# Keshav-Madhav/3d-spatial-sim-for-boid-and-nbody

Hardware: AMD Instinct MI355X
Metric: body-steps/sec (N-body Barnes-Hut, theta=0.5) (higher is better)
Workload: dtype f64 pair forces for the waves of 64 bodies whose densest quarter has G*rho*dt^2 > tau - and for every wave while most of the system qualifies (entered above a third of the waves, left below a quarter; library default 'auto') -, f32 pair forces with f64 sums for the others; f64 opening-test ties, f64; 1 GPU; galaxy_1m_bh; distribution=galaxy, bodies_per_gpu=1000000, bodies_total=1000000, method=barnes_hut, force_precision=auto, parallelism=single GPU

## Files before the change

### 3d-spatial-sim-for-boid-and-nbody_amd/csrc/nbmi.hip

```cpp
#include <math.h>
#include <stdarg.h>
#include <stddef.h>
#include <stdlib.h>
#include <string.h>

#include <algorithm>
#include <type_traits>
#include <utility>
#include <vector>

#include "../../include/nbmi.h"
#include "common.h"
#include "radix_hist.h"
#include "hilbert.h"
#include "visible.h"

namespace nbmi {
static thread_local char g_err[512] = "";
void set_error(const char *fmt, ...) {
    va_list ap;
    va_start(ap, fmt);
    vsnprintf(g_err, sizeof(g_err), fmt, ap);
    va_end(ap);
}
// ... 125 lines not shown

template <bool kHilbert, typename TD, typename TN>
__device__ __forceinline__ uint64_t key_word(double px, double py, double pz, double &cx, double &cy, double &cz, double &hs,
                                             unsigned &st, const TD *hd, const TN *hn) {
    uint64_t kk = 0;
    for (int l = 0; l < 21; l++) {
        const double q = hs * 0.5;
        const bool bx = px >= cx, by = py >= cy, bz = pz >= cz;
        cx = bx ? cx + q : cx - q;
        cy = by ? cy + q : cy - q;
        cz = bz ? cz + q : cz - q;
        hs = q;
        const unsigned oct = (bx ? 1u : 0u) | (by ? 2u : 0u) | (bz ? 4u : 0u);
        if (kHilbert) {
            kk = (kk << 3) | (uint64_t)((hd[st] >> (3u * oct)) & 7u);
            st = (unsigned)(hn[st] >> (5u * oct)) & 31u;
        } else {
            kk = (kk << 3) | (uint64_t)oct;
        }
    }
    return kk;
}

__device__ __noinline__ uint64_t key_low_word(bool hilbert, double px, double py, double pz, double bounds) {
    double cx = 0.0, cy = 0.0, cz = 0.0, hs = bounds;
    unsigned st = 0u;
    if (hilbert) {
        (void)key_word<true>(px, py, pz, cx, cy, cz, hs, st, nbmi::kHilDigit, nbmi::kHilNext);
        return key_word<true>(px, py, pz, cx, cy, cz, hs, st, nbmi::kHilDigit, nbmi::kHilNext);
    }
    (void)key_word<false>(px, py, pz, cx, cy, cz, hs, st, nbmi::kHilDigit, nbmi::kHilNext);
    return key_word<false>(px, py, pz, cx, cy, cz, hs, st, nbmi::kHilDigit, nbmi::kHilNext);
}
__device__ __forceinline__ uint64_t low_word_of(const uint64_t *__restrict__ key_lo, const Bodies &cur, uint32_t b, int hilbert,
                                                const TreeInfo *info) {
    return key_lo ? key_lo[b] : key_low_word(hilbert != 0, cur.x[b], cur.y[b], cur.z[b], info->bounds);
}

constexpr int kKeysHistBlock = 1024, kKeysHistMaxGrid = 512;
constexpr int kKeysHistCounters = 4096;
static inline bool fused_hist_pays(int64_t n) { return n <= 2097152; }
static inline int keys_hist_grid(int64_t n) {
    const int64_t g = (n + 2 * kKeysHistBlock - 1) / (2 * kKeysHistBlock);
    return (int)(g < 1 ? 1 : (g > kKeysHistMaxGrid ? kKeysHistMaxGrid : g));
}
template <bool kHilbert, bool kLean>
__device__ __forceinline__ uint64_t keys_of_body(int64_t i, const double *__restrict__ x, const double *__restrict__ y,
                                                 const double *__restrict__ z, double bounds, uint64_t *__restrict__ key_hi,
                                                 uint64_t *__restrict__ key_lo, uint32_t *__restrict__ idx,
                                                 uint64_t *__restrict__ packed, int shift, const uint32_t *hd, const uint64_t *hn) {
    const double px = x[i], py = y[i], pz = z[i];
    double cx = 0.0, cy = 0.0, cz = 0.0, hs = bounds;
    uint64_t k[2];
    unsigned st = 0u;
    k[0] = key_word<kHilbert>(px, py, pz, cx, cy, cz, hs, st, hd, hn);
// ... 122 lines not shown
    }
    const int64_t s = lo_ok, e = hi_bad;
    if (r == s && e - s > 64 && !(!kPacked && dead_rank && srt[e - 1] == ~0ull)) atomicMax(&info->max_run, (int)(e - s < 0x7fffffff ? e - s : 0x7fffffff));
    uint64_t la = key_lo ? key_lo[p] : 0ull;
    bool have_la = key_lo != nullptr;
    int64_t before = 0;
    for (int64_t j = s; j < e; j++) {
        const uint32_t pj = body(j);
        const uint64_t hj = upper(j, pj);
        if (hj != h) {
            before += hj < h ? 1 : 0;
        } else {
            if (pj == p) continue;
            if (!have_la) { la = low_word_of(key_lo, cur, p, hilbert, info); have_la = true; }
            const uint64_t lj = low_word_of(key_lo, cur, pj, hilbert, info);
            before += (lj < la || (lj == la && pj < p)) ? 1 : 0;
        }
    }
    perm_out[s + before] = p;
    hi_out[s + before] = h;
}

constexpr int kScanItems = 8;
constexpr int kScanTile = kBlock * kScanItems;
constexpr int kSubShift = 11;
static_assert(kScanTile == (1 << kSubShift), "a sub-tile is one workgroup's tile");

struct dd {
    double h, l;
};
__device__ __forceinline__ dd dd_add(const dd &a, const dd &b) {
    const double s = a.h + b.h;
    const double bb = s - a.h;
    double e = (a.h - (s - bb)) + (b.h - bb);
    e += a.l + b.l;
    const double h = s + e;
    return dd{h, e - (h - s)};
}
__device__ __forceinline__ double dd_diff(const dd &a, const dd &b) {
    const dd d = dd_add(a, dd{-b.h, -b.l});
    return d.h + d.l;
}

__device__ __forceinline__ int64_t pex_at(const int32_t *__restrict__ PexL, const int32_t *__restrict__ subPex, int64_t r) {
    return (int64_t)subPex[r >> kSubShift] + PexL[r];
}

struct Mom4 {
    double m, x, y, z;
    int c;
};
__device__ __forceinline__ Mom4 operator+(const Mom4 &a, const Mom4 &b) { return Mom4{a.m + b.m, a.x + b.x, a.y + b.y, a.z + b.z, a.c + b.c}; }
__device__ __forceinline__ Mom4 lane_up(const Mom4 &v, int d) {
    return Mom4{__shfl_up(v.m, d), __shfl_up(v.x, d), __shfl_up(v.y, d), __shfl_up(v.z, d), __shfl_up(v.c, d)};
}

template <int CTRL>
__device__ __forceinline__ float dpp_f(float v) {
    return __int_as_float(__builtin_amdgcn_update_dpp(0, __float_as_int(v), CTRL, 0xF, 0xF, false));
}
__device__ __forceinline__ float add_f(float a, float b) { return a + b; }

template <bool kLean>
__global__ __launch_bounds__(kBlock) void k_gather_scan(Bodies cur, const uint32_t *__restrict__ perm,
                                                        const uint64_t *__restrict__ hi_s, const uint64_t *__restrict__ key_lo,
                                                        int64_t n, double G, float4 *__restrict__ posm_s,
                                                        double4 *__restrict__ p64_s , uint64_t *__restrict__ lo_s,
                                                        int32_t *__restrict__ delta, double4 *__restrict__ S,
                                                        int32_t *__restrict__ PexL, double4 *__restrict__ sub_tot,
                                                        int32_t *__restrict__ sub_cnt, unsigned char *__restrict__ wave_flag,
                                                        int32_t *__restrict__ sub_flag, float dens_thr, float edge_floor,
                                                        const TreeInfo *__restrict__ info, int hilbert) {
    __shared__ int wflag[kBlock / 64];
    int nflag = 0;
    __shared__ int dl[kBlock + 1];
    const int t = threadIdx.x, lane = t & 63, w = t >> 6;
    Mom4 carry{0.0, 0.0, 0.0, 0.0, 0};
#pragma unroll 1
    for (int k = 0; k < kScanItems; k++) {
        const int64_t r0 = (int64_t)blockIdx.x * kScanTile + (int64_t)k * kBlock;
        if (r0 > n) break;
        const int64_t r = r0 + t;
        Mom4 v{0.0, 0.0, 0.0, 0.0, 0};
        int d = -1;
        uint64_t h = 0, l = 0;
        float fx = 0.f, fy = 0.f, fz = 0.f;
        if (r < n) {
            const uint32_t j = perm[r];
            const double x = cur.x[j], y = cur.y[j], z = cur.z[j], gm = G * cur.m[j];
            fx = (float)x; fy = (float)y; fz = (float)z;
            posm_s[r] = make_float4((float)x, (float)y, (float)z, (float)gm);
            if (p64_s) p64_s[r] = make_double4(x, y, z, gm);
            h = hi_s[r];
            if (!kLean) {
                l = key_lo[j];
                lo_s[r] = l;
            }
            if (r + 1 < n) {
                const uint64_t hn = hi_s[r + 1];
                uint64_t ln = 0ull;
                uint64_t lr = l;
                if (hn == h) {
                    if (kLean) lr = low_word_of(nullptr, cur, j, hilbert, info);
                    ln = kLean ? low_word_of(nullptr, cur, perm[r + 1], hilbert, info) : key_lo[perm[r + 1]];
                }
                d = cpl_digits(h, lr, hn, ln);
            }
            delta[r] = d;
            v = Mom4{gm, gm * x, gm * y, gm * z, 0};
        }
        if (wave_flag) {
            const bool have = r < n;
            const float big = 3.0e38f;
            float lox = have ? fx : big, hix = have ? fx : -big, loy = have ? fy : big, hiy = have ? fy : -big;
            float loz = have ? fz : big, hiz = have ? fz : -big, gsum = have ? (float)v.m : 0.f;
#define NBMI_ROW16(V, OP)                      \
    V = OP(V, dpp_f<0xB1>(V));                 \
    V = OP(V, dpp_f<0x4E>(V));                 \
    V = OP(V, dpp_f<0x141>(V));                \
    V = OP(V, dpp_f<0x140>(V));
            NBMI_ROW16(lox, fminf) NBMI_ROW16(hix, fmaxf) NBMI_ROW16(loy, fminf) NBMI_ROW16(hiy, fmaxf)
            NBMI_ROW16(loz, fminf) NBMI_ROW16(hiz, fmaxf) NBMI_ROW16(gsum, add_f)
#undef NBMI_ROW16
            const float vol = fmaxf(hix - lox, edge_floor) * fmaxf(hiy - loy, edge_floor) * fmaxf(hiz - loz, edge_floor);
            float dens = gsum > 0.f ? gsum / vol : 0.f;
            dens = fmaxf(dens, __shfl_xor(dens, 16));
            dens = fmaxf(dens, __shfl_xor(dens, 32));
            const int flag = dens > dens_thr ? 1 : 0;
            if (lane == 0) {
                if (r0 + 64 * w < n) wave_flag[(r0 >> 6) + w] = (unsigned char)flag;
                nflag += (r0 + 64 * w < n) ? flag : 0;
            }
        }
        dl[t + 1] = d;
        if (t == 0) {
            int dp = -1;
            if (r > 0 && r < n) {
                const uint64_t hp = hi_s[r - 1];
                uint64_t lp = 0ull, lr = l;
                if (hp == h) {
                    if (kLean) lr = low_word_of(nullptr, cur, perm[r], hilbert, info);
                    lp = kLean ? low_word_of(nullptr, cur, perm[r - 1], hilbert, info) : key_lo[perm[r - 1]];
                }
                dp = cpl_digits(hp, lp, h, lr);
            }
            dl[0] = dp;
        }
        __syncthreads();
        if (r < n) {
            const int dp = dl[t];
            v.c = d > dp ? d - dp : 0;
        }
        const scan::Scanned<Mom4> sc = scan::block_scan<kBlock>(v, carry, scan::Sum());
        carry = carry + sc.total;
        if (r <= n) {
            S[r] = make_double4(sc.excl.m, sc.excl.x, sc.excl.y, sc.excl.z);
            PexL[r] = sc.excl.c;
        }
    }
    if (wave_flag) {
        if (lane == 0) wflag[w] = nflag;
        __syncthreads();
    }
    if (t == 0) {
        sub_tot[blockIdx.x] = make_double4(carry.m, carry.x, carry.y, carry.z);
        sub_cnt[blockIdx.x] = carry.c;
        if (wave_flag) sub_flag[blockIdx.x] = wflag[0] + wflag[1] + wflag[2] + wflag[3];
    }
}

constexpr int kSubScanThreads = 1024;
struct SubVal {
    dd m, x, y, z;
    long long c;
};
__device__ __forceinline__ SubVal operator+(const SubVal &a, const SubVal &b) {
    return SubVal{dd_add(a.m, b.m), dd_add(a.x, b.x), dd_add(a.y, b.y), dd_add(a.z, b.z), a.c + b.c};
}
__device__ __forceinline__ SubVal sub_zero() { return SubVal{{0.0, 0.0}, {0.0, 0.0}, {0.0, 0.0}, {0.0, 0.0}, 0}; }
__device__ __forceinline__ dd dd_shfl_up(const dd &v, int d) { return dd{__shfl_up(v.h, d), __shfl_up(v.l, d)}; }
__device__ __forceinline__ SubVal lane_up(const SubVal &v, int d) {
    return SubVal{dd_shfl_up(v.m, d), dd_shfl_up(v.x, d), dd_shfl_up(v.y, d), dd_shfl_up(v.z, d), __shfl_up(v.c, d)};
}
constexpr int kAll64Enter = 333, kAll64Leave = 250;
__host__ __device__ inline int all64_rule(int prev, long long ask, long long waves, int enter_pm, int leave_pm) {
    return prev ? (1000 * ask >= (long long)leave_pm * waves ? 1 : 0) : (1000 * ask > (long long)enter_pm * waves ? 1 : 0);
}
__global__ void k_set_all64(TreeInfo *info, int v) { info->force_all64 = v; }

__global__ __launch_bounds__(kSubScanThreads) void k_scan_subtiles(const double4 *__restrict__ sub_tot,
// ... 46 lines not shown
                                              double &M, double &mx, double &my, double &mz) {
    const double4 s0 = S[r], s1 = S[e];
    M = s1.x - s0.x; mx = s1.y - s0.y; my = s1.z - s0.z; mz = s1.w - s0.w;
    const int64_t ur = r >> kSubShift, ue = e >> kSubShift;
    if (ue != ur) {
        const Moment a = T[ur], b = T[ue];
        M += dd_diff(dd{b.m, b.ml}, dd{a.m, a.ml});
        mx += dd_diff(dd{b.x, b.xl}, dd{a.x, a.xl});
        my += dd_diff(dd{b.y, b.yl}, dd{a.y, a.yl});
        mz += dd_diff(dd{b.z, b.zl}, dd{a.z, a.zl});
    }
}

__device__ __forceinline__ void write_sentinel(Node *__restrict__ nodes, int32_t *__restrict__ node_ref, int64_t total,
                                               int64_t link_base = 0) {
    Node sn;
    sn.cx = sn.cy = sn.cz = 1.0e30f;
    sn.gm = 0.f; sn.s2t = 0.f;
    sn.next_off = (unsigned)(total + link_base) * kNodeBytes;
    nodes[total] = sn;
    if (node_ref) node_ref[total] = -1;
}

template <int TILE>
__global__ __launch_bounds__(kBlock) void k_emit_tile(const int32_t *__restrict__ delta, const int32_t *__restrict__ PexL,
                                                      const int32_t *__restrict__ subPex, const double4 *__restrict__ S,
                                                      const Moment *__restrict__ T, const float4 *__restrict__ posm_s,
                                                      const uint64_t *__restrict__ hi_s,
                                                      const uint64_t *__restrict__ lo_s, int64_t n, int64_t capacity,
                                                      double eps, double inv_theta2, Node *__restrict__ nodes,
                                                      Node64 *__restrict__ nodes64, uint8_t *__restrict__ node_level,
                                                      int32_t *__restrict__ node_ref, double4 *__restrict__ diag64,
                                                      NodeD *__restrict__ nodesd , Bodies cur,
                                                      const uint32_t *__restrict__ perm, double G, TreeInfo *info, int hilbert,
                                                      int64_t link_base ) {
    __shared__ uint8_t tree[2 * TILE];
    __shared__ uint8_t dprev;
    __shared__ uint32_t cells[(2 * TILE)];
    const int t = threadIdx.x;
    const int64_t base = (int64_t)blockIdx.x * TILE;
    const int64_t total = n + pex_at(PexL, subPex, n);
    if (blockIdx.x == 0 && t == 0) {
        info->num_nodes = total;
        info->walk_nodes = total;
        info->band2 = 2u * band_half_ulps(__longlong_as_double((long long)info->maxabs_bits), eps);
        if (total + 1 > capacity) {
            info->error = 1;
            if (info->sticky_error == 0) {
                info->sticky_error = 1;
                info->sticky_nodes = total;
            }
        } else {
            write_sentinel(nodes, node_ref, total, link_base);
            if (nodesd) nodesd[total] = NodeD{1.0e30, 1.0e30, 1.0e30, 0.0, 0.0f, (unsigned)(total + link_base) * kNodeDBytes};
        }
    }
    if (total + 1 > capacity) return;
    for (int i = t; i < TILE; i += kBlock) {
        const int64_t r = base + i;
        tree[TILE + i] = (uint8_t)((r < n ? delta[r] : -1) + 1);
    }
    if (t == 0) dprev = (uint8_t)((base > 0 ? delta[base - 1] : -1) + 1);
    __syncthreads();
    for (int width = TILE / 2; width >= 1; width >>= 1) {
        for (int i = t; i < width; i += kBlock) {
            const uint8_t a = tree[2 * (width + i)], b = tree[2 * (width + i) + 1];
            tree[width + i] = a < b ? a : b;
        }
        __syncthreads();
    }
    const int64_t q_tile = pex_at(PexL, subPex, base < n ? base : n);
    const int64_t tile_end = base + TILE < n ? base + TILE : n;
    const int64_t ncell = pex_at(PexL, subPex, tile_end) - q_tile;
    const int64_t nnode = (tile_end - base) + ncell;
    const int64_t idx0 = base + q_tile;
    const double bounds = info->bounds;
    const unsigned bandk = band_half_ulps(__longlong_as_double((long long)info->maxabs_bits), eps);
    for (int64_t c0 = 0; c0 < nnode; c0 += (2 * TILE)) {
        for (int i = t; i < TILE; i += kBlock) {
            const int64_t r = base + i;
            if (r >= n) break;
            const int d = (int)tree[TILE + i] - 1;
            const int dp = (int)(i > 0 ? tree[TILE + i - 1] : dprev) - 1;
            const int cnt = d > dp ? d - dp : 0;
            const int64_t s0 = i + (pex_at(PexL, subPex, r) - q_tile) - c0;
            for (int k = 0; k <= cnt; k++) {
                const int64_t c = s0 + k;
                if (c >= 0 && c < (2 * TILE)) cells[c] = ((uint32_t)i << 6) | (uint32_t)k;
            }
        }
        __syncthreads();
        const int64_t here = nnode - c0 < (2 * TILE) ? nnode - c0 : (2 * TILE);
        for (int64_t c = t; c < here; c += kBlock) {
            const uint32_t cl = cells[c];
            const int i = (int)(cl >> 6), k = (int)(cl & 63u);
            const int64_t r = base + i;
            const int64_t idx = idx0 + c0 + c;
            const int d = (int)tree[TILE + i] - 1;
            const int dp = (int)(i > 0 ? tree[TILE + i - 1] : dprev) - 1;
            const int cnt = d > dp ? d - dp : 0;
            if (k == cnt) {
                const float4 p = posm_s[r];
                Node lf;
                lf.cx = p.x; lf.cy = p.y; lf.cz = p.z; lf.gm = p.w;
                lf.s2t = 0.0f;
                lf.next_off = (unsigned)(idx + 1 + link_base) * kNodeBytes;
                nodes[idx] = lf;
                if (diag64) {
                    const uint32_t j = perm[r];
                    diag64[idx] = make_double4(cur.x[j], cur.y[j], cur.z[j], G * cur.m[j]);
                }
                if (nodesd) {
                    const uint32_t j = perm[r];
                    nodesd[idx] = NodeD{cur.x[j], cur.y[j], cur.z[j], G * cur.m[j], 0.0f, (unsigned)(idx + 1 + link_base) * kNodeDBytes};
                }
                if (node_ref) {
                    node_ref[idx] = (int32_t)r;
                    node_level[idx] = (uint8_t)((d > dp ? d : dp) + 1);
                }
                continue;
            }
            const int lev = dp + 1 + k;
            unsigned h = (unsigned)(TILE + i);
            bool found = false;
            for (;;) {
                if ((int)tree[h] <= lev) { found = true; break; }
                while ((h & 1u) && h > 1u) h >>= 1;
                if (h == 1u) break;
                h += 1u;
            }
            int64_t e;
            if (found) {
                while (h < (unsigned)TILE) {
                    h <<= 1;
                    if ((int)tree[h] > lev) h += 1u;
                }
                e = base + (int64_t)(h - (unsigned)TILE) + 1;
            } else {
                const uint64_t kh = hi_s[r];
                const bool deep = lev > 21;
                const uint64_t kl = lo_s ? lo_s[r] : (deep ? low_word_of(nullptr, cur, perm[r], hilbert, info) : 0ull);
                auto reaches = [&](int64_t u) {
                    const uint64_t hu = hi_s[u];
                    const uint64_t lu = lo_s ? lo_s[u] : (deep && hu == kh ? low_word_of(nullptr, cur, perm[u], hilbert, info) : 0ull);
                    return cpl_digits(kh, kl, hu, lu) >= lev;
                };
                int64_t ok = base + TILE - 1, bad, step = 1;
                for (;;) {
                    const int64_t u = ok + step;
                    if (u >= n) { bad = n; break; }
                    if (reaches(u)) { ok = u; step <<= 1; }
                    else { bad = u; break; }
                }
                while (bad - ok > 1) {
                    const int64_t mid = ok + ((bad - ok) >> 1);
                    if (reaches(mid)) ok = mid; else bad = mid;
                }
                e = bad;
            }
            double M, mx, my, mz;
            range_moments(S, T, r, e, M, mx, my, mz);
            double cx = 0.0, cy = 0.0, cz = 0.0;
            if (M > 0.0) { cx = mx / M; cy = my / M; cz = mz / M; }
            const double size = ldexp(bounds, 1 - lev);
            Node nd;
            nd.cx = (float)cx; nd.cy = (float)cy; nd.cz = (float)cz;
            nd.gm = (float)M;
            const float s2t = (float)(size * size * inv_theta2);
            nd.s2t = __int_as_float(__float_as_int(s2t) + (int)bandk);
            const int64_t nxt = e + pex_at(PexL, subPex, e) + link_base;
            nd.next_off = (unsigned)nxt * kNodeBytes;
            nodes[idx] = nd;
            if (nodesd) nodesd[idx] = NodeD{cx, cy, cz, M, __int_as_float(__float_as_int(s2t) + (int)kBand64), (unsigned)nxt * kNodeDBytes};
            nodes64[idx] = Node64{cx, cy, cz, ldexp(bounds, -lev)};
            if (diag64) diag64[idx] = make_double4(cx, cy, cz, M);
            if (node_ref) {
                node_ref[idx] = (int32_t)r;
                node_level[idx] = (uint8_t)lev;
            }
        }
        __syncthreads();
    }
}

__global__ __launch_bounds__(kBlock) void k_max_level(const int32_t *__restrict__ delta, int64_t n, TreeInfo *info) {
    __shared__ int red[kBlock / 64];
    int m = -1;
    for (int64_t i = (int64_t)blockIdx.x * kBlock + threadIdx.x; i < n; i += (int64_t)gridDim.x * kBlock) {
        const int d = delta[i];
        m = d > m ? d : m;
    }
#pragma unroll
    for (int o = 32; o > 0; o >>= 1) {
        const int other = __shfl_xor(m, o);
        m = other > m ? other : m;
    }
    if ((threadIdx.x & 63) == 0) red[threadIdx.x >> 6] = m;
    __syncthreads();
    if (threadIdx.x == 0) {
        for (int w = 1; w < kBlock / 64; w++) m = red[w] > m ? red[w] : m;
        atomicMax(&info->max_level, m + 1);
// ... 2808 lines not shown
    uint32_t *vis_slot = nullptr, *vis_tiles = nullptr;
    int xcd_chunk = 0;
    int xcd_balance = 1;
    int *xcd_bounds = nullptr;
    unsigned *wave_cycles = nullptr;
    unsigned char *wave_flag = nullptr;
    int32_t *sub_flag = nullptr;
    double step_dt = 0.0;
    double uniform_gm = -1.0;
    double max_gm = 0.0;
    int owner_all64 = -1;
    double owner_dt = 0.0;
    int balance_blocks = 0;
    hipStream_t side = nullptr;
    hipEvent_t ev_walked = nullptr, ev_cut = nullptr;
    bool cut_pending = false;
    int walk_block = kBlock;
    bool keys_lean = true;
    bool lean_build = false;
    bool sort_packed = true;
    uint64_t *packed = nullptr, *packed_s = nullptr;
    nbmi::RadixConfig sort_cfg;
    int sort_fused_hist = -1;
    int sort_bits = 0;
    bool maxabs_fused = false;
    bool fuse_maxabs = true;
    bool hilbert = true;
    double *diag_phi = nullptr;
    int32_t *diag_cnt = nullptr;
    double *diag_part = nullptr;
    long long *diag_partc = nullptr;
    double4 *diag_pot = nullptr;
    TreeInfo *side_info = nullptr;
    double *knn_r2 = nullptr, *knn_mass = nullptr;
    double4 *knn_rows = nullptr;
    unsigned long long *knn_evals = nullptr;
    int32_t *fof_parent = nullptr, *fof_root = nullptr, *fof_minid = nullptr, *fof_cnt = nullptr;
    uint32_t *fof_wleaf = nullptr;
    unsigned long long *fof_counters = nullptr;
    bool fof_ready = false, fof_cat_ready = false;
    uint32_t *fof_key_s = nullptr, *fof_rank = nullptr, *fof_rank_s = nullptr, *fof_tiles = nullptr;
    int32_t *fof_hpos = nullptr, *fof_slot = nullptr, *fof_qhead = nullptr;
    char *fof_sort_tmp = nullptr;
    size_t fof_sort_bytes = 0;
    double *fof_last = nullptr, *fof_first = nullptr;
    int64_t fof_row_cap = 0;
// ... 184 lines not shown
                k_keys_hist<decltype(h)::value, decltype(l)::value><<<grid, kKeysHistBlock, 0, st>>>(
                    cur.x, cur.y, cur.z, n, s->info, s->key_hi, s->key_lo, pk, shift, hist, rounds);
            }
            else
                k_keys<decltype(h)::value, decltype(l)::value><<<nblocks(n), kBlock, 0, st>>>(cur.x, cur.y, cur.z, n, s->info, s->key_hi,
                                                                                             s->key_lo, s->idx, dead, pk, shift);
        });
    });
    if (req.timed) NBMI_HIP_CHECK(hipEventRecord(s->ev[1], st));
    if (packed) {
        NBMI_HIP_CHECK(nbmi::radix_sort_keys_u64(s->tmp_sort, s->tmp_sort_bytes, s->packed, s->packed_s, (size_t)n, kPackIdxBits,
                                                 kPackIdxBits + s->sort_bits, st, s->sort_cfg, fused));
        k_tiefix<true><<<nblocks(n), kBlock, 0, st>>>(s->packed_s, s->key_hi, key_lo, nullptr, shift, s->perm, s->hi_s, n, s->info, cur, hil);
    } else {
        NBMI_HIP_CHECK(nbmi::radix_sort_pairs_u64(s->tmp_sort, s->tmp_sort_bytes, s->key_hi, s->hi_s, s->idx, s->perm,
                                                  (size_t)n, shift, 63, st));
        k_tiefix<false><<<nblocks(n), kBlock, 0, st>>>(s->hi_s, nullptr, key_lo, s->perm, shift, s->idx, s->key_hi, n, s->info, cur, hil,
                                                       dead ? s->let_scan : nullptr, n - n_live);
        std::swap(s->perm, s->idx);
        std::swap(s->hi_s, s->key_hi);
    }
    s->t_hi = s->hi_s;
    if (req.timed) NBMI_HIP_CHECK(hipEventRecord(s->ev[2], st));
    with_bool(lean, [&](auto l) {
        k_gather_scan<decltype(l)::value><<<(int)((n_live + 1 + kScanTile - 1) / kScanTile), kBlock, 0, st>>>(
            cur, s->perm, s->hi_s, key_lo, n_live, s->G, s->posm_s, s->p64_s, lean ? nullptr : s->lo_s, s->delta, s->S, s->Pex,
            s->sub_tot, s->sub_cnt, auto_prec(s) ? s->wave_flag : nullptr, s->sub_flag,
            auto_prec(s) ? (float)(s->prec_tau / (s->step_dt * s->step_dt)) : 0.f, (float)s->softening, s->info, hil);
    });
    return 0;
}

int enqueue_global_tree(nbmi_sim *s, bool aux = true, double4 *diag = nullptr) {
    const int64_t n = s->nt;
    hipStream_t st = s->stream;
    const int64_t nsub = (n + 1 + kScanTile - 1) / kScanTile;
    k_scan_subtiles<<<1, kSubScanThreads, 0, st>>>(s->sub_tot, s->sub_cnt, nsub, s->T, s->subPex,
                                                   auto_prec(s) ? s->sub_flag : nullptr, (n + 63) / 64, s->all64_enter_pm, s->all64_leave_pm, s->info);
    const double inv_theta2 = s->theta > 0.0 ? 1.0 / (s->theta * s->theta) : INFINITY;
    const int64_t ob = s->own_base;
    const bool quad = s->multipole == NBMI_MULTIPOLE_QUADRUPOLE;
    if (quad) {
        aux = true;
        if (!diag) diag = s->quad_pot;
    }
    with_int<kEmitTileSmall, kEmitTile>(n <= kEmitSmallBodies ? kEmitTileSmall : kEmitTile, [&](auto tile) {
        constexpr int kTile = decltype(tile)::value;
        k_emit_tile<kTile><<<(int)((n + kTile - 1) / kTile), kBlock, 0, st>>>(
            s->delta, s->Pex, s->subPex, s->S, s->T, s->t_posm, s->t_hi, s->lean_build ? nullptr : s->t_lo, n,
            s->own_node_rows, s->softening, inv_theta2, s->nodes + ob, s->nodes64 + ob, aux ? s->node_level : nullptr,
            aux ? s->node_ref : nullptr, diag, s->force_prec != 1 && s->nodesd ? s->nodesd + ob : nullptr,
            s->buf[s->curbuf], s->perm, s->G, s->info, s->hilbert ? 1 : 0, ob);
    });
    if (quad && n > 0) {
        k_max_level<<<64, kBlock, 0, st>>>(s->delta, n, s->info);
        for (int lev = kMaxLevel; lev >= 0; lev--)
            k_quad_level<<<kQuadGrid, kBlock, 0, st>>>(s->nodes, s->node_level, diag, s->info, lev, s->quad_work, s->nodesq);
    }
    NBMI_HIP_CHECK(hipGetLastError());
    return 0;
}

int enqueue_tree(nbmi_sim *s, const BuildRequest &req = {}) {
    if (s->owner) {
        nbmi::set_error("this handle is in owner mode: use the nbmi_owner_* calls");
        return NBMI_ERR_ARG;
    }
    const DtScope dt_scope(s, req.step_dt);
    const bool timed = req.timing != BuildTiming::kNone;
    if (req.timing == BuildTiming::kAll) NBMI_HIP_CHECK(hipEventRecord(s->ev[0], s->stream));
    if (int rc = enqueue_maxabs(s)) return rc;
    const bool lean = s->keys_lean && req.step_dt > 0.0 && !req.aux && s->multipole != NBMI_MULTIPOLE_QUADRUPOLE;
    if (int rc = enqueue_local_sort(s, SortRequest{timed, lean})) return rc;
    if (int rc = enqueue_global_tree(s, req.aux, req.diag_rows)) return rc;
    if (timed) NBMI_HIP_CHECK(hipEventRecord(s->ev[3], s->stream));
// ... 304 lines not shown
    if (s->h_info) (void)hipHostFree(s->h_info);
    if (s->stream) (void)hipStreamDestroy(s->stream);
    delete s;
}

static const char *multipole_refusal(const nbmi_sim *s) {
    if (s->method != NBMI_METHOD_BARNES_HUT) return "direct N^2 handles have no cells";
    if (s->owner) return "owner-mode handles are not supported (the exchanged tree rows carry no second moments)";
    if (s->shard_begin != 0 || s->shard_end != s->n) return "sharded handles are not supported (the exchange rows carry no second moments)";
    return nullptr;
}

static void read_env_knobs(nbmi_sim *s) {
    if (const char *e = getenv("NBMI_XCD_CHUNK")) s->xcd_chunk = atoi(e);
    if (const char *e = getenv("NBMI_XCD_BALANCE")) s->xcd_balance = atoi(e);
    if (const char *e = getenv("NBMI_SPLIT_WAVES")) s->split_max_waves = atoll(e);
    if (const char *e = getenv("NBMI_WALK_PAIR")) s->walk_pair = atoi(e);
    if (const char *e = getenv("NBMI_FUSE_MAXABS")) s->fuse_maxabs = atoi(e) != 0;
    if (const char *e = getenv("NBMI_HILBERT")) s->hilbert = atoi(e) != 0;
    if (const char *e = getenv("NBMI_SORT_PACKED")) s->sort_packed = atoi(e) != 0;
    if (const char *e = getenv("NBMI_SORT_DIGIT_BITS")) s->sort_cfg.digit_bits = atoi(e);
    if (const char *e = getenv("NBMI_SORT_THREADS")) s->sort_cfg.threads = atoi(e);
    if (const char *e = getenv("NBMI_SORT_FUSED_HIST")) s->sort_fused_hist = atoi(e) != 0 ? 1 : 0;
    if (const char *e = getenv("NBMI_KEYS_LEAN")) s->keys_lean = atoi(e) != 0;
    if (const char *e = getenv("NBMI_PAIRS_CELLS")) s->pair_cells = atoi(e) != 0;
    if (const char *e = getenv("NBMI_FORCE_PREC")) {
        const int v = atoi(e);
        if (v >= 0 && v <= 2) s->force_prec = v;
    }
    if (const char *e = getenv("NBMI_PREC_TAU")) s->prec_tau = atof(e);
    if (const char *e = getenv("NBMI_MULTIPOLE")) {
        if (!strcmp(e, "quadrupole") || !strcmp(e, "1")) s->multipole_env = NBMI_MULTIPOLE_QUADRUPOLE;
    }
    if (const char *e = getenv("NBMI_ALL64_ENTER")) s->all64_enter_pm = (int)(1000.0 * atof(e) + 0.5);
    if (const char *e = getenv("NBMI_ALL64_LEAVE")) s->all64_leave_pm = (int)(1000.0 * atof(e) + 0.5);
    if (const char *e = getenv("NBMI_SORT_BITS")) {
        const int b = atoi(e);
        if (b >= 8 && b <= 63) s->sort_bits = b;
    }
    if (const char *e = getenv("NBMI_WALK_BLOCK")) {
        const int b = atoi(e);
        if (b == 64 || b == 128 || b == 256) s->walk_block = b;
    }
}

static nbmi_sim *create_failed(nbmi_sim *s) {
    std::string keep = nbmi::get_error();
    nbmi_destroy(s);
    nbmi::set_error("%s", keep.c_str());
    return nullptr;
}

static int create_impl(nbmi_sim *s, const double *pos, const double *vel, const double *mass) {
    const int64_t n = s->n;
    const int64_t c = s->cap > n ? s->cap : n;
    if (!nbmi::radix_config_ok(s->sort_cfg)) {
        nbmi::set_error("NBMI_SORT_DIGIT_BITS must be 8 or 10 and NBMI_SORT_THREADS 256, 512 or 1024 (got %d, %d)", s->sort_cfg.digit_bits,
                        s->sort_cfg.threads);
        return NBMI_ERR_ARG;
    }
    NBMI_HIP_CHECK(hipSetDevice(s->device));
    NBMI_HIP_CHECK(hipStreamCreateWithFlags(&s->stream, hipStreamNonBlocking));
    for (auto &e : s->ev) NBMI_HIP_CHECK(hipEventCreate(&e));
    if (alloc_bodies(s, &s->buf[0], c) || alloc_bodies(s, &s->buf[1], c)) return -2;
    if (dev_alloc(s, &s->posm_s, c) || dev_alloc(s, &s->colors, 3 * (c ? c : 1)) || dev_alloc(s, &s->info, 1)) return -2;
    void *stage = nullptr;
    NBMI_HIP_CHECK(hipMalloc(&stage, (size_t)(c ? c : 1) * 7 * sizeof(double)));
    s->allocs.push_back(stage);
    s->stage = stage;
    NBMI_HIP_CHECK(hipMemsetAsync(s->info, 0, sizeof(TreeInfo), s->stream));
    NBMI_HIP_CHECK(hipMemsetAsync(s->colors, 0, (size_t)(c ? c : 1) * 3 * sizeof(float), s->stream));
    if (s->method == NBMI_METHOD_BARNES_HUT) {
        s->node_capacity = node_rows_for(c) + s->node_extra;
        const int64_t own_rows = node_rows_for(c);
        if (dev_alloc(s, &s->key_hi, c) || dev_alloc(s, &s->key_lo, c) || dev_alloc(s, &s->hi_s, c) ||
            dev_alloc(s, &s->lo_s, c) ||
            (s->sort_packed && !s->owner && (dev_alloc(s, &s->packed, c) || dev_alloc(s, &s->packed_s, c))) || (s->owner && dev_alloc(s, &s->p64_s, c)) || dev_alloc(s, &s->idx, c) ||
            dev_alloc(s, &s->perm, c) || dev_alloc(s, &s->delta, c) || dev_alloc(s, &s->Pex, c + 1) ||
// ... 1701 lines not shown
```

### 3d-spatial-sim-for-boid-and-nbody_amd/csrc/scan.h

```cpp
#pragma once
#include <hip/hip_runtime.h>
#include <stdint.h>

namespace scan {

struct Sum {
    template <class T>
    __device__ T operator()(const T &a, const T &b) const { return a + b; }
};
struct Min {
    template <class T>
    __device__ T operator()(const T &a, const T &b) const { return b < a ? b : a; }
};

template <class T>
__device__ __forceinline__ T lane_up(const T &v, int d) { return __shfl_up(v, d); }

template <class T>
struct Scanned {
    T excl, incl, total;
};

template <int NT, class T, class Op>
__device__ __forceinline__ Scanned<T> block_scan(const T &v, const T &seed, Op op) {
    static_assert(NT % 64 == 0 && NT <= 1024, "whole waves of one workgroup");
    __shared__ T wave_total[NT / 64];
    const int lane = threadIdx.x & 63;
    const int wave = __builtin_amdgcn_readfirstlane(threadIdx.x >> 6);
    T inc = v;
#pragma unroll
    for (int d = 1; d < 64; d <<= 1) {
        const T below = lane_up(inc, d);
        if (lane >= d) inc = op(below, inc);
    }
    if (lane == 63) wave_total[wave] = inc;
    __syncthreads();
    T front = seed, total = wave_total[0];
#pragma unroll
    for (int q = 0; q < NT / 64; q++) {
        if (q < wave) front = op(front, wave_total[q]);
        if (q > 0) total = op(total, wave_total[q]);
    }
    __syncthreads();
    inc = op(front, inc);
    T ex = lane_up(inc, 1);
    if (lane == 0) ex = front;
    return Scanned<T>{ex, inc, total};
}

constexpr int kScanThreads = 1024;
template <class TI, class TO, class Op>
static __global__ __launch_bounds__(kScanThreads) void k_scan_values(const TI *in, TO *out, int64_t m, int64_t stride,
                                                                    TO ident, Op op) {
    in += (int64_t)blockIdx.y * stride;
    out += (int64_t)blockIdx.y * stride;
    TO carry = ident;
    for (int64_t base = 0; base < m; base += kScanThreads) {
        const int64_t i = base + threadIdx.x;
        const TO v = i < m ? (TO)in[i] : ident;
        const Scanned<TO> s = block_scan<kScanThreads>(v, carry, op);
        if (i < m) out[i] = s.excl;
        carry = op(carry, s.total);
    }
    if (threadIdx.x == 0) out[m] = carry;
}

template <int NT, class TO>
__device__ __forceinline__ int64_t tile_slot(const TO *__restrict__ tile_off, unsigned c) {
    return (int64_t)tile_off[blockIdx.x] + block_scan<NT>(c, 0u, Sum()).excl;
}
// ... 47 lines not shown
```

Baseline: 516.0 million body-steps/s.

## Widen gather-scan to 1024 threads and drop shared delta exchange

The gather/scan kernel is templated on block size and defaults to 1024 threads, so one sub-tile is covered in two rounds instead of eight. It uses a new round-aware block scan that keeps wave totals in shared memory across rounds. The previous-delta exchange through shared memory and its extra barrier is replaced by a lane shuffle, with lane 0 computing its own predecessor. The low Morton/Hilbert word is recomputed by an inlined single 42-level loop, the emit kernel takes a packed argument struct with wave-uniform scalars, and occupancy hints are added. This risks higher register pressure and a different floating-point summation order in the moment scan.

```diff
diff --git a/3d-spatial-sim-for-boid-and-nbody_amd/csrc/nbmi.hip b/3d-spatial-sim-for-boid-and-nbody_amd/csrc/nbmi.hip
--- a/3d-spatial-sim-for-boid-and-nbody_amd/csrc/nbmi.hip
+++ b/3d-spatial-sim-for-boid-and-nbody_amd/csrc/nbmi.hip
@@ -171,15 +171,30 @@
     return kk;
 }
 
-__device__ __noinline__ uint64_t key_low_word(bool hilbert, double px, double py, double pz, double bounds) {
+__device__ __forceinline__ uint64_t key_low_word_inl(bool hilbert, double px, double py, double pz, double bounds) {
     double cx = 0.0, cy = 0.0, cz = 0.0, hs = bounds;
     unsigned st = 0u;
-    if (hilbert) {
-        (void)key_word<true>(px, py, pz, cx, cy, cz, hs, st, nbmi::kHilDigit, nbmi::kHilNext);
-        return key_word<true>(px, py, pz, cx, cy, cz, hs, st, nbmi::kHilDigit, nbmi::kHilNext);
-    }
-    (void)key_word<false>(px, py, pz, cx, cy, cz, hs, st, nbmi::kHilDigit, nbmi::kHilNext);
-    return key_word<false>(px, py, pz, cx, cy, cz, hs, st, nbmi::kHilDigit, nbmi::kHilNext);
+    uint64_t kk = 0;
+#pragma unroll 1
+    for (int l = 0; l < 42; l++) {
+        const double q = hs * 0.5;
+        const bool bx = px >= cx, by = py >= cy, bz = pz >= cz;
+        cx = bx ? cx + q : cx - q;
+        cy = by ? cy + q : cy - q;
+        cz = bz ? cz + q : cz - q;
+        hs = q;
+        const unsigned oct = (bx ? 1u : 0u) | (by ? 2u : 0u) | (bz ? 4u : 0u);
+        unsigned digit = oct;
+        if (hilbert) {
+            digit = (nbmi::kHilDigit[st] >> (3u * oct)) & 7u;
+            st = (unsigned)(nbmi::kHilNext[st] >> (5u * oct)) & 31u;
+        }
+        kk = (kk << 3) | (uint64_t)digit;
+    }
+    return kk & 0x7fffffffffffffffull;
+}
+__device__ __noinline__ uint64_t key_low_word(bool hilbert, double px, double py, double pz, double bounds) {
+    return key_low_word_inl(hilbert, px, py, pz, bounds);
 }
 __device__ __forceinline__ uint64_t low_word_of(const uint64_t *__restrict__ key_lo, const Bodies &cur, uint32_t b, int hilbert,
                                                 const TreeInfo *info) {
@@ -348,6 +363,7 @@
 }
 
 constexpr int kScanItems = 8;
+constexpr int kScanWide = 1024;
 constexpr int kScanTile = kBlock * kScanItems;
 constexpr int kSubShift = 11;
 static_assert(kScanTile == (1 << kSubShift), "a sub-tile is one workgroup's tile");
@@ -380,6 +396,13 @@
 __device__ __forceinline__ Mom4 lane_up(const Mom4 &v, int d) {
     return Mom4{__shfl_up(v.m, d), __shfl_up(v.x, d), __shfl_up(v.y, d), __shfl_up(v.z, d), __shfl_up(v.c, d)};
 }
+__device__ __forceinline__ double readlane_f64(double v, int src) {
+    return __hiloint2double(__builtin_amdgcn_readlane(__double2hiint(v), src), __builtin_amdgcn_readlane(__double2loint(v), src));
+}
+__device__ __forceinline__ Mom4 lane_get(const Mom4 &v, int src) {
+    return Mom4{readlane_f64(v.m, src), readlane_f64(v.x, src), readlane_f64(v.y, src), readlane_f64(v.z, src),
+                __builtin_amdgcn_readlane(v.c, src)};
+}
 
 template <int CTRL>
 __device__ __forceinline__ float dpp_f(float v) {
@@ -387,53 +410,60 @@
 }
 __device__ __forceinline__ float add_f(float a, float b) { return a + b; }
 
-template <bool kLean>
-__global__ __launch_bounds__(kBlock) void k_gather_scan(Bodies cur, const uint32_t *__restrict__ perm,
-                                                        const uint64_t *__restrict__ hi_s, const uint64_t *__restrict__ key_lo,
-                                                        int64_t n, double G, float4 *__restrict__ posm_s,
-                                                        double4 *__restrict__ p64_s , uint64_t *__restrict__ lo_s,
-                                                        int32_t *__restrict__ delta, double4 *__restrict__ S,
-                                                        int32_t *__restrict__ PexL, double4 *__restrict__ sub_tot,
-                                                        int32_t *__restrict__ sub_cnt, unsigned char *__restrict__ wave_flag,
-                                                        int32_t *__restrict__ sub_flag, float dens_thr, float edge_floor,
-                                                        const TreeInfo *__restrict__ info, int hilbert) {
-    __shared__ int wflag[kBlock / 64];
+template <bool kLean, int NT>
+__global__ __launch_bounds__(NT) __attribute__((amdgpu_waves_per_eu(kLean || NT == kScanWide ? 8 : 7, 8))) void k_gather_scan(
+    Bodies cur, const uint32_t *__restrict__ perm, const uint64_t *__restrict__ hi_s, const uint64_t *__restrict__ key_lo,
+    int64_t n, double G, float4 *__restrict__ posm_s, double4 *__restrict__ p64_s ,
+    uint64_t *__restrict__ lo_s, int32_t *__restrict__ delta, double4 *__restrict__ S, int32_t *__restrict__ PexL,
+    double4 *__restrict__ sub_tot, int32_t *__restrict__ sub_cnt, unsigned char *__restrict__ wave_flag,
+    int32_t *__restrict__ sub_flag, float dens_thr, float edge_floor, const TreeInfo *__restrict__ info, int hilbert) {
+    __shared__ int wflag[NT / 64];
     int nflag = 0;
-    __shared__ int dl[kBlock + 1];
     const int t = threadIdx.x, lane = t & 63, w = t >> 6;
     Mom4 carry{0.0, 0.0, 0.0, 0.0, 0};
 #pragma unroll 1
-    for (int k = 0; k < kScanItems; k++) {
-        const int64_t r0 = (int64_t)blockIdx.x * kScanTile + (int64_t)k * kBlock;
+    for (int k = 0; k < kScanTile / NT; k++) {
+        const int64_t r0 = (int64_t)blockIdx.x * kScanTile + (int64_t)k * NT;
         if (r0 > n) break;
         const int64_t r = r0 + t;
         Mom4 v{0.0, 0.0, 0.0, 0.0, 0};
-        int d = -1;
-        uint64_t h = 0, l = 0;
+        int d = -1, dp = -1;
         float fx = 0.f, fy = 0.f, fz = 0.f;
         if (r < n) {
+            const bool nxt = r + 1 < n, prv = lane == 0 && r > 0;
             const uint32_t j = perm[r];
+            const uint64_t h = hi_s[r], hn = nxt ? hi_s[r + 1] : 0ull, hp = prv ? hi_s[r - 1] : 0ull;
             const double x = cur.x[j], y = cur.y[j], z = cur.z[j], gm = G * cur.m[j];
-            fx = (float)x; fy = (float)y; fz = (float)z;
-            posm_s[r] = make_float4((float)x, (float)y, (float)z, (float)gm);
-            if (p64_s) p64_s[r] = make_double4(x, y, z, gm);
-            h = hi_s[r];
+            uint64_t l = 0ull;
             if (!kLean) {
                 l = key_lo[j];
                 lo_s[r] = l;
             }
-            if (r + 1 < n) {
-                const uint64_t hn = hi_s[r + 1];
-                uint64_t ln = 0ull;
-                uint64_t lr = l;
-                if (hn == h) {
-                    if (kLean) lr = low_word_of(nullptr, cur, j, hilbert, info);
-                    ln = kLean ? low_word_of(nullptr, cur, perm[r + 1], hilbert, info) : key_lo[perm[r + 1]];
+            fx = (float)x; fy = (float)y; fz = (float)z;
+            posm_s[r] = make_float4((float)x, (float)y, (float)z, (float)gm);
+            if (p64_s) p64_s[r] = make_double4(x, y, z, gm);
+            v = Mom4{gm, gm * x, gm * y, gm * z, 0};
+            const bool eq_n = nxt && hn == h, eq_p = prv && hp == h;
+            uint64_t ln = 0ull, lp = 0ull;
+            if (eq_n || eq_p) {
+                if (kLean) {
+                    const bool hil = hilbert != 0;
+                    const double bounds = info->bounds;
+#pragma unroll 1
+                    for (int side = -1; side < 2; side++) {
+                        if (!(side < 0 ? eq_p : (side > 0 ? eq_n : true))) continue;
+                        const uint32_t b = perm[r + side];
+                        const uint64_t lb = key_low_word_inl(hil, cur.x[b], cur.y[b], cur.z[b], bounds);
+                        if (side < 0) lp = lb; else if (side > 0) ln = lb; else l = lb;
+                    }
+                } else {
+                    if (eq_n) ln = key_lo[perm[r + 1]];
+                    if (eq_p) lp = key_lo[perm[r - 1]];
                 }
-                d = cpl_digits(h, lr, hn, ln);
             }
+            if (nxt) d = cpl_digits(h, l, hn, ln);
+            if (prv) dp = cpl_digits(hp, lp, h, l);
             delta[r] = d;
-            v = Mom4{gm, gm * x, gm * y, gm * z, 0};
         }
         if (wave_flag) {
             const bool have = r < n;
@@ -458,27 +488,12 @@
                 nflag += (r0 + 64 * w < n) ? flag : 0;
             }
         }
-        dl[t + 1] = d;
-        if (t == 0) {
-            int dp = -1;
-            if (r > 0 && r < n) {
-                const uint64_t hp = hi_s[r - 1];
-                uint64_t lp = 0ull, lr = l;
-                if (hp == h) {
-                    if (kLean) lr = low_word_of(nullptr, cur, perm[r], hilbert, info);
-                    lp = kLean ? low_word_of(nullptr, cur, perm[r - 1], hilbert, info) : key_lo[perm[r - 1]];
-                }
-                dp = cpl_digits(hp, lp, h, lr);
-            }
-            dl[0] = dp;
-        }
-        __syncthreads();
-        if (r < n) {
-            const int dp = dl[t];
-            v.c = d > dp ? d - dp : 0;
-        }
-        const scan::Scanned<Mom4> sc = scan::block_scan<kBlock>(v, carry, scan::Sum());
-        carry = carry + sc.total;
+        const int d_below = __shfl_up(d, 1);
+        if (lane != 0) dp = d_below;
+        if (r < n) v.c = d > dp ? d - dp : 0;
+        const scan::ScannedRounds<Mom4> sc =
+            scan::block_scan_rounds256<NT, kScanTile / NT>(v, Mom4{0.0, 0.0, 0.0, 0.0, 0}, scan::Sum(), k);
+        carry = sc.carry;
         if (r <= n) {
             S[r] = make_double4(sc.excl.m, sc.excl.x, sc.excl.y, sc.excl.z);
             PexL[r] = sc.excl.c;
@@ -491,7 +506,11 @@
     if (t == 0) {
         sub_tot[blockIdx.x] = make_double4(carry.m, carry.x, carry.y, carry.z);
         sub_cnt[blockIdx.x] = carry.c;
-        if (wave_flag) sub_flag[blockIdx.x] = wflag[0] + wflag[1] + wflag[2] + wflag[3];
+        if (wave_flag) {
+            int f = 0;
+            for (int q = 0; q < NT / 64; q++) f += wflag[q];
+            sub_flag[blockIdx.x] = f;
+        }
     }
 }
 
@@ -584,76 +603,126 @@
     if (node_ref) node_ref[total] = -1;
 }
 
+struct EmitArgs {
+    const int32_t *delta, *PexL, *subPex;
+    const double4 *S;
+    const Moment *T;
+    const float4 *posm_s;
+    const uint64_t *hi_s, *lo_s;
+    int64_t n, capacity;
+    double eps, inv_theta2;
+    Node *nodes;
+    Node64 *nodes64;
+    uint8_t *node_level;
+    int32_t *node_ref;
+    double4 *diag64;
+    NodeD *nodesd;
+    Bodies cur;
+    const uint32_t *perm;
+    double G;
+    TreeInfo *info;
+    int hilbert;
+    int64_t link_base;
+};
+
+__device__ __forceinline__ int64_t first_lane(int64_t v) {
+    const unsigned lo = __builtin_amdgcn_readfirstlane((unsigned)v), hi = __builtin_amdgcn_readfirstlane((unsigned)((uint64_t)v >> 32));
+    return (int64_t)(((uint64_t)hi << 32) | lo);
+}
+
+__device__ __forceinline__ void emit_header(const EmitArgs &a, int64_t total) {
+    TreeInfo *info = a.info;
+    info->num_nodes = total;
+    info->walk_nodes = total;
+    info->band2 = 2u * band_half_ulps(__longlong_as_double((long long)info->maxabs_bits), a.eps);
+    if (total + 1 > a.capacity) {
+        info->error = 1;
+        if (info->sticky_error == 0) {
+            info->sticky_error = 1;
+            info->sticky_nodes = total;
+        }
+    } else {
+        write_sentinel(a.nodes, a.node_ref, total, a.link_base);
+        if (a.nodesd) a.nodesd[total] = NodeD{1.0e30, 1.0e30, 1.0e30, 0.0, 0.0f, (unsigned)(total + a.link_base) * kNodeDBytes};
+    }
+}
+
+__device__ __forceinline__ int64_t cell_end_beyond(const EmitArgs &a, int64_t r, int lev, int64_t ok) {
+    const uint64_t *hi_s = a.hi_s, *lo_s = a.lo_s;
+    const int64_t n = a.n;
+    const uint64_t kh = hi_s[r];
+    const bool deep = lev > 21;
+    auto recomputed = [&](int64_t u) {
+        const uint32_t b = a.perm[u];
+        return key_low_word_inl(a.hilbert != 0, a.cur.x[b], a.cur.y[b], a.cur.z[b], a.info->bounds);
+    };
+    const uint64_t kl = lo_s ? lo_s[r] : (deep ? recomputed(r) : 0ull);
+    auto reaches = [&](int64_t u) {
+        const uint64_t hu = hi_s[u];
+        const uint64_t lu = lo_s ? lo_s[u] : (deep && hu == kh ? recomputed(u) : 0ull);
+        return cpl_digits(kh, kl, hu, lu) >= lev;
+    };
+    int64_t bad, step = 1;
+    for (;;) {
+        const int64_t u = ok + step;
+        if (u >= n) { bad = n; break; }
+        if (reaches(u)) { ok = u; step <<= 1; }
+        else { bad = u; break; }
+    }
+    while (bad - ok > 1) {
+        const int64_t mid = ok + ((bad - ok) >> 1);
+        if (reaches(mid)) ok = mid; else bad = mid;
+    }
+    return bad;
+}
+
 template <int TILE>
-__global__ __launch_bounds__(kBlock) void k_emit_tile(const int32_t *__restrict__ delta, const int32_t *__restrict__ PexL,
-                                                      const int32_t *__restrict__ subPex, const double4 *__restrict__ S,
-                                                      const Moment *__restrict__ T, const float4 *__restrict__ posm_s,
-                                                      const uint64_t *__restrict__ hi_s,
-                                                      const uint64_t *__restrict__ lo_s, int64_t n, int64_t capacity,
-                                                      double eps, double inv_theta2, Node *__restrict__ nodes,
-                                                      Node64 *__restrict__ nodes64, uint8_t *__restrict__ node_level,
-                                                      int32_t *__restrict__ node_ref, double4 *__restrict__ diag64,
-                                                      NodeD *__restrict__ nodesd , Bodies cur,
-                                                      const uint32_t *__restrict__ perm, double G, TreeInfo *info, int hilbert,
-                                                      int64_t link_base ) {
+__global__ __launch_bounds__(kBlock) __attribute__((amdgpu_waves_per_eu(5, 8))) void k_emit_tile(const EmitArgs a) {
     __shared__ uint8_t tree[2 * TILE];
     __shared__ uint8_t dprev;
     __shared__ uint32_t cells[(2 * TILE)];
     const int t = threadIdx.x;
+    const int64_t n = a.n;
     const int64_t base = (int64_t)blockIdx.x * TILE;
-    const int64_t total = n + pex_at(PexL, subPex, n);
-    if (blockIdx.x == 0 && t == 0) {
-        info->num_nodes = total;
-        info->walk_nodes = total;
-        info->band2 = 2u * band_half_ulps(__longlong_as_double((long long)info->maxabs_bits), eps);
-        if (total + 1 > capacity) {
-            info->error = 1;
-            if (info->sticky_error == 0) {
-                info->sticky_error = 1;
-                info->sticky_nodes = total;
-            }
-        } else {
-            write_sentinel(nodes, node_ref, total, link_base);
-            if (nodesd) nodesd[total] = NodeD{1.0e30, 1.0e30, 1.0e30, 0.0, 0.0f, (unsigned)(total + link_base) * kNodeDBytes};
-        }
-    }
-    if (total + 1 > capacity) return;
+    const int64_t total = first_lane(n + pex_at(a.PexL, a.subPex, n));
+    if (blockIdx.x == 0 && t == 0) emit_header(a, total);
+    if (total + 1 > a.capacity) return;
     for (int i = t; i < TILE; i += kBlock) {
         const int64_t r = base + i;
-        tree[TILE + i] = (uint8_t)((r < n ? delta[r] : -1) + 1);
-    }
-    if (t == 0) dprev = (uint8_t)((base > 0 ? delta[base - 1] : -1) + 1);
+        tree[TILE + i] = (uint8_t)((r < n ? a.delta[r] : -1) + 1);
+    }
+    if (t == 0) dprev = (uint8_t)((base > 0 ? a.delta[base - 1] : -1) + 1);
     __syncthreads();
     for (int width = TILE / 2; width >= 1; width >>= 1) {
         for (int i = t; i < width; i += kBlock) {
-            const uint8_t a = tree[2 * (width + i)], b = tree[2 * (width + i) + 1];
-            tree[width + i] = a < b ? a : b;
+            const uint8_t a0 = tree[2 * (width + i)], a1 = tree[2 * (width + i) + 1];
+            tree[width + i] = a0 < a1 ? a0 : a1;
         }
         __syncthreads();
     }
-    const int64_t q_tile = pex_at(PexL, subPex, base < n ? base : n);
+    const int64_t q_tile = first_lane(pex_at(a.PexL, a.subPex, base < n ? base : n));
     const int64_t tile_end = base + TILE < n ? base + TILE : n;
-    const int64_t ncell = pex_at(PexL, subPex, tile_end) - q_tile;
-    const int64_t nnode = (tile_end - base) + ncell;
+    const int ncell = (int)(first_lane(pex_at(a.PexL, a.subPex, tile_end)) - q_tile);
+    const int nnode = (int)(tile_end - base) + ncell;
     const int64_t idx0 = base + q_tile;
-    const double bounds = info->bounds;
-    const unsigned bandk = band_half_ulps(__longlong_as_double((long long)info->maxabs_bits), eps);
-    for (int64_t c0 = 0; c0 < nnode; c0 += (2 * TILE)) {
+    const double bounds = a.info->bounds;
+    const unsigned bandk = band_half_ulps(__longlong_as_double((long long)a.info->maxabs_bits), a.eps);
+    for (int c0 = 0; c0 < nnode; c0 += (2 * TILE)) {
         for (int i = t; i < TILE; i += kBlock) {
             const int64_t r = base + i;
             if (r >= n) break;
             const int d = (int)tree[TILE + i] - 1;
             const int dp = (int)(i > 0 ? tree[TILE + i - 1] : dprev) - 1;
             const int cnt = d > dp ? d - dp : 0;
-            const int64_t s0 = i + (pex_at(PexL, subPex, r) - q_tile) - c0;
+            const int s0 = i + (int)(pex_at(a.PexL, a.subPex, r) - q_tile) - c0;
             for (int k = 0; k <= cnt; k++) {
-                const int64_t c = s0 + k;
+                const int c = s0 + k;
                 if (c >= 0 && c < (2 * TILE)) cells[c] = ((uint32_t)i << 6) | (uint32_t)k;
             }
         }
         __syncthreads();
-        const int64_t here = nnode - c0 < (2 * TILE) ? nnode - c0 : (2 * TILE);
-        for (int64_t c = t; c < here; c += kBlock) {
+        const int here = nnode - c0 < (2 * TILE) ? nnode - c0 : (2 * TILE);
+        for (int c = t; c < here; c += kBlock) {
             const uint32_t cl = cells[c];
             const int i = (int)(cl >> 6), k = (int)(cl & 63u);
             const int64_t r = base + i;
@@ -662,23 +731,23 @@
             const int dp = (int)(i > 0 ? tree[TILE + i - 1] : dprev) - 1;
             const int cnt = d > dp ? d - dp : 0;
             if (k == cnt) {
-                const float4 p = posm_s[r];
+                const float4 p = a.posm_s[r];
                 Node lf;
                 lf.cx = p.x; lf.cy = p.y; lf.cz = p.z; lf.gm = p.w;
                 lf.s2t = 0.0f;
-                lf.next_off = (unsigned)(idx + 1 + link_base) * kNodeBytes;
-                nodes[idx] = lf;
-                if (diag64) {
-                    const uint32_t j = perm[r];
-                    diag64[idx] = make_double4(cur.x[j], cur.y[j], cur.z[j], G * cur.m[j]);
+                lf.next_off = (unsigned)(idx + 1 + a.link_base) * kNodeBytes;
+                a.nodes[idx] = lf;
+                if (a.diag64) {
+                    const uint32_t j = a.perm[r];
+                    a.diag64[idx] = make_double4(a.cur.x[j], a.cur.y[j], a.cur.z[j], a.G * a.cur.m[j]);
                 }
-                if (nodesd) {
-                    const uint32_t j = perm[r];
-                    nodesd[idx] = NodeD{cur.x[j], cur.y[j], cur.z[j], G * cur.m[j], 0.0f, (unsigned)(idx + 1 + link_base) * kNodeDBytes};
+                if (a.nodesd) {
+                    const uint32_t j = a.perm[r];
+                    a.nodesd[idx] = NodeD{a.cur.x[j], a.cur.y[j], a.cur.z[j], a.G * a.cur.m[j], 0.0f, (unsigned)(idx + 1 + a.link_base) * kNodeDBytes};
                 }
-                if (node_ref) {
-                    node_ref[idx] = (int32_t)r;
-                    node_level[idx] = (uint8_t)((d > dp ? d : dp) + 1);
+                if (a.node_ref) {
+                    a.node_ref[idx] = (int32_t)r;
+                    a.node_level[idx] = (uint8_t)((d > dp ? d : dp) + 1);
                 }
                 continue;
             }
@@ -699,46 +768,27 @@
                 }
                 e = base + (int64_t)(h - (unsigned)TILE) + 1;
             } else {
-                const uint64_t kh = hi_s[r];
-                const bool deep = lev > 21;
-                const uint64_t kl = lo_s ? lo_s[r] : (deep ? low_word_of(nullptr, cur, perm[r], hilbert, info) : 0ull);
-                auto reaches = [&](int64_t u) {
-                    const uint64_t hu = hi_s[u];
-                    const uint64_t lu = lo_s ? lo_s[u] : (deep && hu == kh ? low_word_of(nullptr, cur, perm[u], hilbert, info) : 0ull);
-                    return cpl_digits(kh, kl, hu, lu) >= lev;
-                };
-                int64_t ok = base + TILE - 1, bad, step = 1;
-                for (;;) {
-                    const int64_t u = ok + step;
-                    if (u >= n) { bad = n; break; }
-                    if (reaches(u)) { ok = u; step <<= 1; }
-                    else { bad = u; break; }
-                }
-                while (bad - ok > 1) {
-                    const int64_t mid = ok + ((bad - ok) >> 1);
-                    if (reaches(mid)) ok = mid; else bad = mid;
-                }
-                e = bad;
+                e = cell_end_beyond(a, r, lev, base + TILE - 1);
             }
             double M, mx, my, mz;
-            range_moments(S, T, r, e, M, mx, my, mz);
+            range_moments(a.S, a.T, r, e, M, mx, my, mz);
             double cx = 0.0, cy = 0.0, cz = 0.0;
             if (M > 0.0) { cx = mx / M; cy = my / M; cz = mz / M; }
             const double size = ldexp(bounds, 1 - lev);
             Node nd;
             nd.cx = (float)cx; nd.cy = (float)cy; nd.cz = (float)cz;
             nd.gm = (float)M;
-            const float s2t = (float)(size * size * inv_theta2);
+            const float s2t = (float)(size * size * a.inv_theta2);
             nd.s2t = __int_as_float(__float_as_int(s2t) + (int)bandk);
-            const int64_t nxt = e + pex_at(PexL, subPex, e) + link_base;
+            const int64_t nxt = e + pex_at(a.PexL, a.subPex, e) + a.link_base;
             nd.next_off = (unsigned)nxt * kNodeBytes;
-            nodes[idx] = nd;
-            if (nodesd) nodesd[idx] = NodeD{cx, cy, cz, M, __int_as_float(__float_as_int(s2t) + (int)kBand64), (unsigned)nxt * kNodeDBytes};
-            nodes64[idx] = Node64{cx, cy, cz, ldexp(bounds, -lev)};
-            if (diag64) diag64[idx] = make_double4(cx, cy, cz, M);
-            if (node_ref) {
-                node_ref[idx] = (int32_t)r;
-                node_level[idx] = (uint8_t)lev;
+            a.nodes[idx] = nd;
+            if (a.nodesd) a.nodesd[idx] = NodeD{cx, cy, cz, M, __int_as_float(__float_as_int(s2t) + (int)kBand64), (unsigned)nxt * kNodeDBytes};
+            a.nodes64[idx] = Node64{cx, cy, cz, ldexp(bounds, -lev)};
+            if (a.diag64) a.diag64[idx] = make_double4(cx, cy, cz, M);
+            if (a.node_ref) {
+                a.node_ref[idx] = (int32_t)r;
+                a.node_level[idx] = (uint8_t)lev;
             }
         }
         __syncthreads();
@@ -3593,6 +3643,7 @@
     uint64_t *packed = nullptr, *packed_s = nullptr;
     nbmi::RadixConfig sort_cfg;
     int sort_fused_hist = -1;
+    int gather_threads = 0;
     int sort_bits = 0;
     bool maxabs_fused = false;
     bool fuse_maxabs = true;
@@ -3823,11 +3874,15 @@
     }
     s->t_hi = s->hi_s;
     if (req.timed) NBMI_HIP_CHECK(hipEventRecord(s->ev[2], st));
+    const int gather_nt = s->gather_threads ? s->gather_threads : kScanWide;
     with_bool(lean, [&](auto l) {
-        k_gather_scan<decltype(l)::value><<<(int)((n_live + 1 + kScanTile - 1) / kScanTile), kBlock, 0, st>>>(
-            cur, s->perm, s->hi_s, key_lo, n_live, s->G, s->posm_s, s->p64_s, lean ? nullptr : s->lo_s, s->delta, s->S, s->Pex,
-            s->sub_tot, s->sub_cnt, auto_prec(s) ? s->wave_flag : nullptr, s->sub_flag,
-            auto_prec(s) ? (float)(s->prec_tau / (s->step_dt * s->step_dt)) : 0.f, (float)s->softening, s->info, hil);
+        with_int<kBlock, kScanWide>(gather_nt, [&](auto nt) {
+            k_gather_scan<decltype(l)::value, decltype(nt)::value>
+                <<<(int)((n_live + 1 + kScanTile - 1) / kScanTile), decltype(nt)::value, 0, st>>>(
+                    cur, s->perm, s->hi_s, key_lo, n_live, s->G, s->posm_s, s->p64_s, lean ? nullptr : s->lo_s, s->delta, s->S,
+                    s->Pex, s->sub_tot, s->sub_cnt, auto_prec(s) ? s->wave_flag : nullptr, s->sub_flag,
+                    auto_prec(s) ? (float)(s->prec_tau / (s->step_dt * s->step_dt)) : 0.f, (float)s->softening, s->info, hil);
+        });
     });
     return 0;
 }
@@ -3847,11 +3902,11 @@
     }
     with_int<kEmitTileSmall, kEmitTile>(n <= kEmitSmallBodies ? kEmitTileSmall : kEmitTile, [&](auto tile) {
         constexpr int kTile = decltype(tile)::value;
-        k_emit_tile<kTile><<<(int)((n + kTile - 1) / kTile), kBlock, 0, st>>>(
+        k_emit_tile<kTile><<<(int)((n + kTile - 1) / kTile), kBlock, 0, st>>>(EmitArgs{
             s->delta, s->Pex, s->subPex, s->S, s->T, s->t_posm, s->t_hi, s->lean_build ? nullptr : s->t_lo, n,
             s->own_node_rows, s->softening, inv_theta2, s->nodes + ob, s->nodes64 + ob, aux ? s->node_level : nullptr,
             aux ? s->node_ref : nullptr, diag, s->force_prec != 1 && s->nodesd ? s->nodesd + ob : nullptr,
-            s->buf[s->curbuf], s->perm, s->G, s->info, s->hilbert ? 1 : 0, ob);
+            s->buf[s->curbuf], s->perm, s->G, s->info, s->hilbert ? 1 : 0, ob});
     });
     if (quad && n > 0) {
         k_max_level<<<64, kBlock, 0, st>>>(s->delta, n, s->info);
@@ -4202,6 +4257,7 @@
     if (const char *e = getenv("NBMI_SORT_DIGIT_BITS")) s->sort_cfg.digit_bits = atoi(e);
     if (const char *e = getenv("NBMI_SORT_THREADS")) s->sort_cfg.threads = atoi(e);
     if (const char *e = getenv("NBMI_SORT_FUSED_HIST")) s->sort_fused_hist = atoi(e) != 0 ? 1 : 0;
+    if (const char *e = getenv("NBMI_GATHER_THREADS")) s->gather_threads = atoi(e);
     if (const char *e = getenv("NBMI_KEYS_LEAN")) s->keys_lean = atoi(e) != 0;
     if (const char *e = getenv("NBMI_PAIRS_CELLS")) s->pair_cells = atoi(e) != 0;
     if (const char *e = getenv("NBMI_FORCE_PREC")) {
@@ -4234,6 +4290,10 @@
 static int create_impl(nbmi_sim *s, const double *pos, const double *vel, const double *mass) {
     const int64_t n = s->n;
     const int64_t c = s->cap > n ? s->cap : n;
+    if (s->gather_threads != 0 && s->gather_threads != kBlock && s->gather_threads != kScanWide) {
+        nbmi::set_error("NBMI_GATHER_THREADS must be 256 or 1024 (got %d)", s->gather_threads);
+        return NBMI_ERR_ARG;
+    }
     if (!nbmi::radix_config_ok(s->sort_cfg)) {
         nbmi::set_error("NBMI_SORT_DIGIT_BITS must be 8 or 10 and NBMI_SORT_THREADS 256, 512 or 1024 (got %d, %d)", s->sort_cfg.digit_bits,
                         s->sort_cfg.threads);
diff --git a/3d-spatial-sim-for-boid-and-nbody_amd/csrc/scan.h b/3d-spatial-sim-for-boid-and-nbody_amd/csrc/scan.h
--- a/3d-spatial-sim-for-boid-and-nbody_amd/csrc/scan.h
+++ b/3d-spatial-sim-for-boid-and-nbody_amd/csrc/scan.h
@@ -46,6 +46,52 @@
     T ex = lane_up(inc, 1);
     if (lane == 0) ex = front;
     return Scanned<T>{ex, inc, total};
+}
+
+template <class T>
+__device__ __forceinline__ T lane_get(const T &v, int src) { return __shfl(v, src); }
+
+template <class T>
+struct ScannedRounds {
+    T excl, incl, carry;
+};
+template <int NT, int ROUNDS, class T, class Op>
+__device__ __forceinline__ ScannedRounds<T> block_scan_rounds256(const T &v, const T &seed, Op op, int round) {
+    static_assert(NT % 256 == 0 && NT <= 1024, "whole groups of 256 threads in one workgroup");
+    constexpr int kGroups = ROUNDS * (NT / 256);
+    static_assert(kGroups <= 64, "one lane per group");
+    __shared__ T wave_total[4 * kGroups];
+    const int lane = threadIdx.x & 63;
+    const int wave = __builtin_amdgcn_readfirstlane(threadIdx.x >> 6);
+    round = __builtin_amdgcn_readfirstlane(round);
+    T inc = v;
+#pragma unroll
+    for (int d = 1; d < 64; d <<= 1) {
+        const T below = lane_up(inc, d);
+        if (lane >= d) inc = op(below, inc);
+    }
+    const int my_wave = round * (NT / 64) + wave, my_group = my_wave >> 2, groups = (round + 1) * (NT / 256);
+    if (lane == 63) wave_total[my_wave] = inc;
+    __syncthreads();
+    T total = seed;
+    if (lane < groups) {
+        total = wave_total[4 * lane];
+#pragma unroll
+        for (int q = 1; q < 4; q++) total = op(total, wave_total[4 * lane + q]);
+    }
+    T carry = seed, front = seed;
+#pragma unroll
+    for (int g = 0; g < kGroups; g++) {
+        if (g == my_group) front = carry;
+        if (g < groups) carry = op(carry, lane_get(total, g));
+    }
+#pragma unroll
+    for (int q = 0; q < 3; q++)
+        if (q < (my_wave & 3)) front = op(front, wave_total[4 * my_group + q]);
+    inc = op(front, inc);
+    T ex = lane_up(inc, 1);
+    if (lane == 0) ex = front;
+    return ScannedRounds<T>{ex, inc, carry};
 }
 
 constexpr int kScanThreads = 1024;
```

New measurement: 519.4 million body-steps/s (median of 6 runs). Within noise of the previous version (+0.6%).
